# pixeli99/SVD_Xtend

Measured on AMD Instinct MI355X. Metric: train-step samples/sec (14-frame 512x320 fp16 SVD UNet), higher is better.
Workload: dtype fp16; 1 GPU; SVD UNet train step, 14 frames 512x320, batch 1/GPU, 1524623082 params (397620480 trainable: temporal_transformer_block*), fwd + EDM loss + bwd + grad all-reduce + AdamW; global_batch=1, grad_accum=1, parallelism=dp1, grad_allreduce=none, ranks_seen=1, allreduce_bytes=1590482176, exec=hipgraph, gemm_tuning_sweeps=0, gemm_variant=4

## Files before the change

svd_xtend_amd/csrc/norm.hip:

```cpp
#include "common.h"
#include <stdlib.h>

namespace {


struct GnGeom {
    int n_s, rows, C, G, cg, cc, rpi;
    int slab;
};

__device__ __forceinline__ void group_sums(const float* stats, int n_s, int n, int G, int g, float i0, float i1, float& s, float& ss) {
    long long a = 0, b = 0;
    const long long* st = reinterpret_cast<const long long*>(stats);
#pragma unroll
    for (int r = 0; r < SVDX_GN_REPLICAS; ++r) {
        const size_t o = (((size_t)r * n_s + n) * G + g) * 2;
        a += st[o]; b += st[o + 1];
    }
    s = (float)a * i0; ss = (float)b * i1;
}
__device__ __forceinline__ void group_mean_rstd(const float* stats, int n_s, int n, int G, int g, float cnt, float eps, float i0, float i1,
                                                float& mean, float& rstd) {
    float s, ss;
    group_sums(stats, n_s, n, G, g, i0, i1, s, ss);
    mean = s / cnt;
    const float var = fmaxf(ss / cnt - mean * mean, 0.f);
    rstd = rsqrtf(var + eps);
}

template <bool BWD>
__device__ __forceinline__ void gn_block_stats(const float* stats, const float* bstats, const GnGeom& q, int n, float eps, float* sm) {
    const int g = threadIdx.x;
    if (g < q.G) {
        int fk0, fk1, bk0, bk1;
        gn_fixed_scales((long)q.rows * q.cg, 0, fk0, fk1);
        const float cnt = (float)q.rows * q.cg;
        float mean, rstd;
        group_mean_rstd(stats, q.n_s, n, q.G, g, cnt, eps, exp2f((float)-fk0), exp2f((float)-fk1), mean, rstd);
        sm[g * 4] = mean; sm[g * 4 + 1] = rstd;
        if (BWD) {
            gn_fixed_scales((long)q.rows * q.cg, 1, bk0, bk1);
            float s1, s2;
            group_sums(bstats, q.n_s, n, q.G, g, exp2f((float)-bk0), exp2f((float)-bk1), s1, s2);
            sm[g * 4 + 2] = s1 / cnt; sm[g * 4 + 3] = s2 / cnt;
        }
    }
    __syncthreads();
}
__device__ __forceinline__ void gn_load8f(const float* p, float (&o)[8]) {
    const f32x4 a = *reinterpret_cast<const f32x4*>(p), b = *reinterpret_cast<const f32x4*>(p + 4);
    o[0] = a[0]; o[1] = a[1]; o[2] = a[2]; o[3] = a[3]; o[4] = b[0]; o[5] = b[1]; o[6] = b[2]; o[7] = b[3];
}

template <typename T, int MODE>
__global__ void gn_reduce_kernel(const T* __restrict__ x, const T* __restrict__ dy, const float* __restrict__ stats,
                                 const float* __restrict__ gamma, const float* __restrict__ beta, float* out,
                                 GnGeom q, float eps, int silu) {
    __shared__ unsigned long long gacc[64];
    __shared__ float sm[32 * 4];
    const int t = threadIdx.x;
    if (t < 64) gacc[t] = 0ull;
    int sk0, sk1;
    gn_fixed_scales((long)q.rows * q.cg, MODE, sk0, sk1);
    const float m0 = exp2f((float)sk0), m1 = exp2f((float)sk1);
    const int n = blockIdx.x, slab = blockIdx.y;
    const int j = t % q.cc, ry = t / q.cc;
    const bool worker = ry < q.rpi;
    const int r0 = slab * q.slab, r1 = min(q.rows, r0 + q.slab);
    constexpr int U = MODE == 0 ? 4 : 2;
    const size_t base = (size_t)n * q.rows * q.C + j * 8;
    Vec8<T> xb[U], db[U], xn[U], dn[U];
    auto fetch = [&](int r, Vec8<T> (&xo)[U], Vec8<T> (&dd)[U]) __attribute__((always_inline)) {
#pragma unroll
        for (int u = 0; u < U; ++u) {
            const int rr = min(r + u * q.rpi, q.rows - 1);
            xo[u] = *reinterpret_cast<const Vec8<T>*>(x + base + (size_t)rr * q.C);
            if (MODE == 1) dd[u] = *reinterpret_cast<const Vec8<T>*>(dy + base + (size_t)rr * q.C);
        }
    };
    int r = r0 + ry;
    if (worker && r < r1) fetch(r, xb, db);
    float a0[8], a1[8];
#pragma unroll
    for (int e = 0; e < 8; ++e) a0[e] = a1[e] = 0.f;
    float sc[8], sh[8], gm[8], mu[8], rs[8];
    if (MODE == 1) {
        gn_block_stats<false>(stats, nullptr, q, n, eps, sm);
        float bt[8];
        gn_load8f(gamma + j * 8, gm);
        gn_load8f(beta + j * 8, bt);
#pragma unroll
        for (int e = 0; e < 8; ++e) {
            const int g = (j * 8 + e) / q.cg;
            mu[e] = sm[g * 4]; rs[e] = sm[g * 4 + 1];
            sc[e] = rs[e] * gm[e];
            sh[e] = bt[e] - mu[e] * sc[e];
        }
    } else {
        __syncthreads();
    }
    if (worker) {
        for (; r < r1; r += U * q.rpi) {
            const int rn = r + U * q.rpi;
            if (rn < r1) fetch(rn, xn, dn);
#pragma unroll
            for (int u = 0; u < U; ++u) {
                if (r + u * q.rpi < r1) {
                    if (MODE == 0) {
#pragma unroll
                        for (int e = 0; e < 8; ++e) { const float xv = to_f<T>(xb[u].v[e]); a0[e] += xv; a1[e] += xv * xv; }
                    } else {
#pragma unroll
                        for (int e = 0; e < 8; ++e) {
                            const float xv = to_f<T>(xb[u].v[e]);
                            float dz = to_f<T>(db[u].v[e]);
                            if (silu) dz *= silu_gradf_(xv * sc[e] + sh[e]);
                            const float dzg = dz * gm[e];
                            a0[e] += dzg;
                            a1[e] += dzg * (xv - mu[e]) * rs[e];
                        }
                    }
                }
            }
#pragma unroll
            for (int u = 0; u < U; ++u) { xb[u] = xn[u]; if (MODE == 1) db[u] = dn[u]; }
        }
        int cur = (j * 8) / q.cg;
        float s0 = 0.f, s1 = 0.f;
#pragma unroll
        for (int e = 0; e < 8; ++e) {
            const int g = (j * 8 + e) / q.cg;
            if (g != cur) {
                atomicAdd(&gacc[cur * 2], (unsigned long long)__float2ll_rn(s0 * m0));
                atomicAdd(&gacc[cur * 2 + 1], (unsigned long long)__float2ll_rn(s1 * m1));
                cur = g; s0 = 0.f; s1 = 0.f;
            }
            s0 += a0[e]; s1 += a1[e];
        }
        atomicAdd(&gacc[cur * 2], (unsigned long long)__float2ll_rn(s0 * m0));
        atomicAdd(&gacc[cur * 2 + 1], (unsigned long long)__float2ll_rn(s1 * m1));
    }
    __syncthreads();
    if (t < 2 * q.G)
        atomicAdd(reinterpret_cast<unsigned long long*>(out) + ((size_t)(slab % SVDX_GN_REPLICAS) * q.n_s + n) * q.G * 2 + t, gacc[t]);
}

template <typename T, int MODE>
__global__ void gn_apply_kernel(const T* __restrict__ x, const T* __restrict__ dy, const float* __restrict__ stats,
                                const float* __restrict__ bstats, const float* __restrict__ gamma,
                                const float* __restrict__ beta, const T* __restrict__ add, T* __restrict__ out,
                                GnGeom q, float eps, int silu) {
    __shared__ float sm[32 * 4];
    const int t = threadIdx.x;
    const int n = blockIdx.x, slab = blockIdx.y;
    const int j = t % q.cc, ry = t / q.cc;
    const bool worker = ry < q.rpi;
    const int r0 = slab * q.slab, r1 = min(q.rows, r0 + q.slab);
    constexpr int U = MODE == 0 ? 4 : 2;
    const size_t base = (size_t)n * q.rows * q.C + j * 8;
    Vec8<T> xb[U], db[U], ab[U], xn[U], dn[U], an[U];
    auto fetch = [&](int r, Vec8<T> (&xo)[U], Vec8<T> (&dd)[U], Vec8<T> (&aa)[U]) __attribute__((always_inline)) {
#pragma unroll
        for (int u = 0; u < U; ++u) {
            const size_t off = base + (size_t)min(r + u * q.rpi, q.rows - 1) * q.C;
            xo[u] = *reinterpret_cast<const Vec8<T>*>(x + off);
            if (MODE == 1) {
                dd[u] = *reinterpret_cast<const Vec8<T>*>(dy + off);
                if (add) aa[u] = *reinterpret_cast<const Vec8<T>*>(add + off);
            }
        }
    };
    int r = r0 + ry;
    if (worker && r < r1) fetch(r, xb, db, ab);
    gn_block_stats<MODE == 1>(stats, bstats, q, n, eps, sm);
    if (!worker) return;
    float sc[8], sh[8], gm[8], mu[8], rs[8], b1[8], b2[8], bt[8];
    gn_load8f(gamma + j * 8, gm);
    gn_load8f(beta + j * 8, bt);
#pragma unroll
    for (int e = 0; e < 8; ++e) {
        const int g = (j * 8 + e) / q.cg;
        mu[e] = sm[g * 4]; rs[e] = sm[g * 4 + 1];
        sc[e] = rs[e] * gm[e];
        sh[e] = bt[e] - mu[e] * sc[e];
        if (MODE == 1) { b1[e] = sm[g * 4 + 2]; b2[e] = sm[g * 4 + 3]; }
    }
    for (; r < r1; r += U * q.rpi) {
        const int rn = r + U * q.rpi;
        if (MODE == 0 && rn < r1) fetch(rn, xn, dn, an);
#pragma unroll
        for (int u = 0; u < U; ++u) {
            const int rr = r + u * q.rpi;
            if (rr < r1) {
                float o[8];
                if (MODE == 0) {
#pragma unroll
                    for (int e = 0; e < 8; ++e) {
                        const float z = to_f<T>(xb[u].v[e]) * sc[e] + sh[e];
                        o[e] = silu ? siluf_(z) : z;
                    }
                } else {
#pragma unroll
                    for (int e = 0; e < 8; ++e) {
                        const float xv = to_f<T>(xb[u].v[e]);
                        float dz = to_f<T>(db[u].v[e]);
                        if (silu) dz *= silu_gradf_(xv * sc[e] + sh[e]);
                        const float xhat = (xv - mu[e]) * rs[e];
                        o[e] = rs[e] * (dz * gm[e] - (b1[e] + xhat * b2[e]));
                        if (add) o[e] += to_f<T>(ab[u].v[e]);
                    }
                }
                store8<T>(out + base + (size_t)rr * q.C, o);
            }
        }
        if (MODE == 0) {
#pragma unroll
            for (int u = 0; u < U; ++u) xb[u] = xn[u];
        } else if (rn < r1) {
            fetch(rn, xb, db, ab);
        }
    }
}

int gn_geom(GnGeom& q, int n_s, int rows, int C, int G, int& threads, bool reduce = false) {
    SVDX_CHECK_ARG(n_s > 0 && rows > 0 && C > 0 && G > 0 && G <= 32, "groupnorm: bad sizes");
    SVDX_CHECK_ARG(C % G == 0 && C % 8 == 0 && C / 8 <= 1024, "groupnorm: C=%d must be a multiple of 8 and of G", C);
    q.n_s = n_s; q.rows = rows; q.C = C; q.G = G; q.cg = C / G; q.cc = C / 8;
    q.rpi = q.cc >= 256 ? 1 : 256 / q.cc;
    threads = q.cc * q.rpi;
    int slab = reduce ? 64 : 32;
    const long want = reduce ? 512 : 1024;
    while (slab > 2 * q.rpi && slab > 2 && (long)n_s * ((rows + slab - 1) / slab) < want) slab >>= 1;
    q.slab = slab;
    return 0;
}

constexpr int LN_MAXCH_LIMIT = 4;

template <typename T, int LN_MAXCH, int R>
__global__ __launch_bounds__(256) void ln_fwd_kernel(const T* __restrict__ x, const float* __restrict__ gamma,
                                                     const float* __restrict__ beta, T* __restrict__ y,
                                                     float* __restrict__ stats, int rows, int C, float eps) {
    const int lane = threadIdx.x & 63;
    const int cc = C / 8;
    const int wid = blockIdx.x * 4 + (threadIdx.x >> 6), nw = gridDim.x * 4;
    const float invC = 1.f / (float)C;
    for (int row0 = wid * R; row0 < rows; row0 += nw * R) {
        Vec8<T> raw[R][LN_MAXCH];
#pragma unroll
        for (int k = 0; k < R; ++k) {
            const int row = min(row0 + k, rows - 1);
#pragma unroll
            for (int i = 0; i < LN_MAXCH; ++i) {
                const int j = lane + i * 64;
                if (j < cc) raw[k][i] = *reinterpret_cast<const Vec8<T>*>(x + (size_t)row * C + j * 8);
            }
        }
#pragma unroll
        for (int k = 0; k < R; ++k) {
            const int row = row0 + k;
            float v[LN_MAXCH][8];
            float s = 0.f;
#pragma unroll
            for (int i = 0; i < LN_MAXCH; ++i) {
                if (lane + i * 64 < cc) {
#pragma unroll
                    for (int e = 0; e < 8; ++e) { v[i][e] = to_f<T>(raw[k][i].v[e]); s += v[i][e]; }
                }
            }
            const float mean = wave_sum(s) * invC;
            float ss = 0.f;
#pragma unroll
            for (int i = 0; i < LN_MAXCH; ++i) {
                if (lane + i * 64 < cc) {
#pragma unroll
                    for (int e = 0; e < 8; ++e) { const float d = v[i][e] - mean; ss += d * d; }
                }
            }
            const float rstd = rsqrtf(wave_sum(ss) * invC + eps);
            if (row < rows) {
                if (lane == 0) { stats[(size_t)row * 2] = mean; stats[(size_t)row * 2 + 1] = rstd; }
#pragma unroll
                for (int i = 0; i < LN_MAXCH; ++i) {
                    const int j = lane + i * 64;
                    if (j < cc) {
                        float o[8];
#pragma unroll
                        for (int e = 0; e < 8; ++e) o[e] = (v[i][e] - mean) * rstd * gamma[j * 8 + e] + beta[j * 8 + e];
                        store8<T>(y + (size_t)row * C + j * 8, o);
                    }
                }
            }
        }
    }
}

template <typename T, int NCH>
__global__ __launch_bounds__(256) void ln_fwd16_kernel(const T* __restrict__ x, const float* __restrict__ gamma, const float* __restrict__ beta,
                                                       T* __restrict__ y, float* __restrict__ stats, int rows, int C, float eps) {
    const int l16 = threadIdx.x & 15, grp = threadIdx.x >> 4;
    const int cc = C / 8;
    float gm[NCH][8], bt[NCH][8];
    bool cv[NCH];
    int cl[NCH];
#pragma unroll
    for (int j = 0; j < NCH; ++j) {
        const int c = l16 + 16 * j;
        cv[j] = c < cc;
        cl[j] = min(c, cc - 1);
        gn_load8f(gamma + cl[j] * 8, gm[j]);
        gn_load8f(beta + cl[j] * 8, bt[j]);
    }
    const float invC = 1.f / (float)C;
    constexpr int R = 2;
    for (int row0 = (blockIdx.x * 16 + grp) * R; row0 < rows; row0 += gridDim.x * 16 * R) {
        Vec8<T> raw[R][NCH];
#pragma unroll
        for (int k = 0; k < R; ++k)
#pragma unroll
            for (int j = 0; j < NCH; ++j) raw[k][j] = *reinterpret_cast<const Vec8<T>*>(x + (size_t)min(row0 + k, rows - 1) * C + cl[j] * 8);
#pragma unroll
        for (int k = 0; k < R; ++k) {
            const int row = row0 + k;
            float v[NCH][8];
            float s = 0.f;
#pragma unroll
            for (int j = 0; j < NCH; ++j)
#pragma unroll
                for (int e = 0; e < 8; ++e) { v[j][e] = cv[j] ? to_f<T>(raw[k][j].v[e]) : 0.f; s += v[j][e]; }
            const float mean = row16_sum(s) * invC;
            float ss = 0.f;
#pragma unroll
            for (int j = 0; j < NCH; ++j)
#pragma unroll
                for (int e = 0; e < 8; ++e) { const float d = cv[j] ? v[j][e] - mean : 0.f; ss += d * d; }
            const float rstd = rsqrtf(row16_sum(ss) * invC + eps);
            if (row < rows) {
                if (l16 == 0) *reinterpret_cast<float2*>(stats + (size_t)row * 2) = float2{mean, rstd};
#pragma unroll
                for (int j = 0; j < NCH; ++j) {
                    if (cv[j]) {
                        float o[8];
#pragma unroll
                        for (int e = 0; e < 8; ++e) o[e] = (v[j][e] - mean) * rstd * gm[j][e] + bt[j][e];
                        store8<T>(y + (size_t)row * C + cl[j] * 8, o);
                    }
                }
            }
        }
    }
}

template <int LANES>
__device__ __forceinline__ float ln_group_sum(float v) {
    v = row16_sum(v);
    if (LANES >= 32) v += __shfl_xor(v, 16, 64);
    if (LANES >= 64) v += __shfl_xor(v, 32, 64);
    return v;
}

template <typename T, int LANES, int NCH, bool AFFINE>
__global__ __launch_bounds__(256, 2) void ln_bwd_kernel(const T* __restrict__ dy, const T* __restrict__ x, const float* __restrict__ stats,
                                                        const float* __restrict__ gamma, const T* __restrict__ add, const T* __restrict__ add2,
                                                        float add2_scale, T* __restrict__ dx, float* dgamma, float* dbeta, float* partial, int rows,
                                                        int C) {
    extern __shared__ float red[];
    constexpr int GROUPS = 256 / LANES;
    const int ll = threadIdx.x % LANES, grp = threadIdx.x / LANES;
    const int cc = C / 8;
    float gm[NCH][8], pg[AFFINE ? NCH : 1][8], pb[AFFINE ? NCH : 1][8];
    bool cv[NCH];
    int cl[NCH];
#pragma unroll
    for (int j = 0; j < NCH; ++j) {
        const int c = ll + LANES * j;
        cv[j] = c < cc;
        cl[j] = min(c, cc - 1);
        gn_load8f(gamma + cl[j] * 8, gm[j]);
        if (AFFINE) {
#pragma unroll
            for (int e = 0; e < 8; ++e) pg[j][e] = pb[j][e] = 0.f;
        }
    }
    const float invC = 1.f / (float)C;
    for (int row = blockIdx.x * GROUPS + grp; row < rows; row += gridDim.x * GROUPS) {
        constexpr bool PRE = !(AFFINE && NCH > 3);
        Vec8<T> xr[NCH], dr[NCH], ar[PRE ? NCH : 1], a2r[PRE ? NCH : 1];
#pragma unroll
        for (int j = 0; j < NCH; ++j) {
            if (cv[j]) {
                const size_t off = (size_t)row * C + cl[j] * 8;
                xr[j] = *reinterpret_cast<const Vec8<T>*>(x + off);
                dr[j] = *reinterpret_cast<const Vec8<T>*>(dy + off);
                if (PRE && add) ar[j] = *reinterpret_cast<const Vec8<T>*>(add + off);
                if (PRE && add2) a2r[j] = *reinterpret_cast<const Vec8<T>*>(add2 + off);
            }
        }
        const float2 mr = *reinterpret_cast<const float2*>(stats + (size_t)row * 2);
        float s1 = 0.f, s2 = 0.f;
#pragma unroll
        for (int j = 0; j < NCH; ++j) {
            if (cv[j]) {
#pragma unroll
                for (int e = 0; e < 8; ++e) {
                    const float d = to_f<T>(dr[j].v[e]);
                    const float xh = (to_f<T>(xr[j].v[e]) - mr.x) * mr.y;
                    const float dg = d * gm[j][e];
                    s1 += dg;
                    s2 += dg * xh;
                    if (AFFINE) {
                        pg[j][e] += d * xh;
                        pb[j][e] += d;
                    }
                }
            }
        }
        const float m1 = ln_group_sum<LANES>(s1) * invC, m2 = ln_group_sum<LANES>(s2) * invC;
#pragma unroll
        for (int j = 0; j < NCH; ++j) {
            if (cv[j]) {
                const size_t off = (size_t)row * C + cl[j] * 8;
                float o[8];
#pragma unroll
                for (int e = 0; e < 8; ++e) {
                    const float xh = (to_f<T>(xr[j].v[e]) - mr.x) * mr.y;
                    o[e] = mr.y * (to_f<T>(dr[j].v[e]) * gm[j][e] - m1 - xh * m2);
                }
                if (add) {
                    const Vec8<T> a8 = PRE ? ar[PRE ? j : 0] : *reinterpret_cast<const Vec8<T>*>(add + off);
#pragma unroll
                    for (int e = 0; e < 8; ++e) o[e] += to_f<T>(a8.v[e]);
                }
                if (add2) {
                    const Vec8<T> a8 = PRE ? a2r[PRE ? j : 0] : *reinterpret_cast<const Vec8<T>*>(add2 + off);
#pragma unroll
                    for (int e = 0; e < 8; ++e) o[e] += add2_scale * to_f<T>(a8.v[e]);
                }
                store8<T>(dx + off, o);
            }
        }
    }
    if (AFFINE) {
        float* mine = red + (size_t)grp * C;
#pragma unroll 1
        for (int which = 0; which < 2; ++which) {
#pragma unroll
            for (int j = 0; j < NCH; ++j) {
                if (cv[j]) {
#pragma unroll
                    for (int e = 0; e < 8; ++e) mine[cl[j] * 8 + e] = which == 0 ? pg[j][e] : pb[j][e];
                }
            }
            __syncthreads();
            for (int i = threadIdx.x; i < C; i += 256) {
                float t = 0.f;
#pragma unroll
                for (int g = 0; g < GROUPS; ++g) t += red[(size_t)g * C + i];
                if (partial) partial[(size_t)blockIdx.x * 2 * C + which * C + i] = t;
                else atomicAdd((which == 0 ? dgamma : dbeta) + i, t);
            }
            __syncthreads();
        }
    }
}

__device__ __forceinline__ void ln_param_reduce_body(const float* __restrict__ partial, int nblk, int C, float* dgamma, float* dbeta,
                                                     int blk, float (*sm)[64]) {
    const int cl = threadIdx.x & 63, rg = threadIdx.x >> 6;
    const int col = blk * 64 + cl;
    float s = 0.f;
    if (col < 2 * C) {
#pragma unroll 8
        for (int b = rg; b < nblk; b += 16) s += partial[(size_t)b * 2 * C + col];
    }
    sm[rg][cl] = s;
    __syncthreads();
    if (rg == 0 && col < 2 * C) {
        float t = 0.f;
#pragma unroll
        for (int i = 0; i < 16; ++i) t += sm[i][cl];
        if (col < C) dgamma[col] += t; else dbeta[col - C] += t;
    }
}

__global__ __launch_bounds__(1024) void ln_param_reduce_kernel(const float* __restrict__ partial, int nblk, int C,
                                                               float* dgamma, float* dbeta) {
    __shared__ float sm[16][64];
    ln_param_reduce_body(partial, nblk, C, dgamma, dbeta, blockIdx.x, sm);
}

struct LnRedPack {
    svdx_lnred_job job[SVDX_BATCH_MAX_JOBS];
    int start[SVDX_BATCH_MAX_JOBS + 1];
    int n_jobs;
};

__global__ __launch_bounds__(1024) void ln_param_reduce_batch_kernel(const LnRedPack pk) {
    __shared__ float sm[16][64];
    int j = 0;
    while (j + 1 < pk.n_jobs && (int)blockIdx.x >= pk.start[j + 1]) ++j;
    const svdx_lnred_job& q = pk.job[j];
    ln_param_reduce_body(q.partial, q.nblk, q.C, q.dgamma, q.dbeta, blockIdx.x - pk.start[j], sm);
}

static int ln_bwd_affine_blocks(int rows, int C) {
    const int cc = C / 8;
    const int lanes = cc <= 48 ? 16 : (cc <= 96 ? 32 : 64);
    const int groups = 256 / lanes;
    const int per = 1;
    const int cap = min(512, SVDX_LN_PARTIAL_ROWS);
    return max(1, min(cdiv(rows, per * groups), cap));
}

}

extern "C" int svdx_ln_bwd_blocks(int rows, int C) { return rows > 0 && C > 0 && C % 8 == 0 ? ln_bwd_affine_blocks(rows, C) : 0; }

extern "C" int svdx_ln_param_reduce_batch(const svdx_lnred_job* jobs, int n_jobs, void* stream) {
    SVDX_CHECK_ARG(jobs && n_jobs > 0, "svdx_ln_param_reduce_batch: bad args");
    for (int j0 = 0; j0 < n_jobs; j0 += SVDX_BATCH_MAX_JOBS) {
        LnRedPack pk;
        pk.n_jobs = min(n_jobs - j0, SVDX_BATCH_MAX_JOBS);
        int blocks = 0;
        for (int j = 0; j < pk.n_jobs; ++j) {
            const svdx_lnred_job& q = jobs[j0 + j];
            SVDX_CHECK_ARG(q.partial && q.dgamma && q.dbeta && q.nblk > 0 && q.C > 0, "svdx_ln_param_reduce_batch: job %d: bad args", j0 + j);
            pk.job[j] = q;
            pk.start[j] = blocks;
            blocks += cdiv(2 * q.C, 64);
        }
        for (int j = pk.n_jobs; j <= SVDX_BATCH_MAX_JOBS; ++j) pk.start[j] = blocks;
        hipLaunchKernelGGL(ln_param_reduce_batch_kernel, dim3(blocks), dim3(1024), 0, (hipStream_t)stream, pk);
        SVDX_LAUNCH_CHECK("svdx_ln_param_reduce_batch");
    }
    return 0;
}

extern "C" int svdx_gn_stats(const void* x, float* stats, int n_s, int rows, int C, int G, int prezeroed, int dtype, void* stream) {
    GnGeom q; int threads;
    if (int rc = gn_geom(q, n_s, rows, C, G, threads, true)) return rc;
    hipStream_t st = (hipStream_t)stream;
    if (!prezeroed) { if (int rc = svdx_zero(stats, sizeof(long long) * 2 * n_s * G * SVDX_GN_REPLICAS, stream)) return rc; }
    dim3 grid(n_s, cdiv(rows, q.slab));
    DISPATCH_DTYPE(dtype, hipLaunchKernelGGL((gn_reduce_kernel<T, 0>), grid, dim3(threads), 0, st, (const T*)x,
                                             (const T*)nullptr, (const float*)nullptr, (const float*)nullptr,
                                             (const float*)nullptr, stats, q, 0.f, 0));
    SVDX_LAUNCH_CHECK("svdx_gn_stats");
    return 0;
}

extern "C" int svdx_gn_apply(const void* x, const float* stats, const float* gamma, const float* beta, void* y,
                             int n_s, int rows, int C, int G, float eps, int silu, int dtype, void* stream) {
    GnGeom q; int threads;
    if (int rc = gn_geom(q, n_s, rows, C, G, threads)) return rc;
    dim3 grid(n_s, cdiv(rows, q.slab));
    DISPATCH_DTYPE(dtype, hipLaunchKernelGGL((gn_apply_kernel<T, 0>), grid, dim3(threads), 0, (hipStream_t)stream,
                                             (const T*)x, (const T*)nullptr, stats, (const float*)nullptr, gamma, beta,
                                             (const T*)nullptr, (T*)y, q, eps, silu));
    SVDX_LAUNCH_CHECK("svdx_gn_apply");
    return 0;
}

extern "C" int svdx_gn_bwd_stats(const void* dy, const void* x, const float* stats, const float* gamma,
                                 const float* beta, float* bstats, int n_s, int rows, int C, int G, float eps,
                                 int silu, int prezeroed, int dtype, void* stream) {
    GnGeom q; int threads;
    if (int rc = gn_geom(q, n_s, rows, C, G, threads, true)) return rc;
    hipStream_t st = (hipStream_t)stream;
    if (!prezeroed) { if (int rc = svdx_zero(bstats, sizeof(long long) * 2 * n_s * G * SVDX_GN_REPLICAS, stream)) return rc; }
    dim3 grid(n_s, cdiv(rows, q.slab));
    DISPATCH_DTYPE(dtype, hipLaunchKernelGGL((gn_reduce_kernel<T, 1>), grid, dim3(threads), 0, st, (const T*)x,
                                             (const T*)dy, stats, gamma, beta, bstats, q, eps, silu));
    SVDX_LAUNCH_CHECK("svdx_gn_bwd_stats");
    return 0;
}

extern "C" int svdx_gn_bwd_apply(const void* dy, const void* x, const float* stats, const float* bstats,
                                 const float* gamma, const float* beta, const void* add, void* dx, int n_s, int rows,
                                 int C, int G, float eps, int silu, int dtype, void* stream) {
    GnGeom q; int threads;
    if (int rc = gn_geom(q, n_s, rows, C, G, threads)) return rc;
    dim3 grid(n_s, cdiv(rows, q.slab));
    DISPATCH_DTYPE(dtype, hipLaunchKernelGGL((gn_apply_kernel<T, 1>), grid, dim3(threads), 0, (hipStream_t)stream,
                                             (const T*)x, (const T*)dy, stats, bstats, gamma, beta, (const T*)add,
                                             (T*)dx, q, eps, silu));
    SVDX_LAUNCH_CHECK("svdx_gn_bwd_apply");
    return 0;
}

extern "C" int svdx_ln_fwd(const void* x, const float* gamma, const float* beta, void* y, float* stats, int rows,
                           int C, float eps, int dtype, void* stream) {
    SVDX_CHECK_ARG(rows > 0 && C % 8 == 0 && C / 8 <= 64 * LN_MAXCH_LIMIT, "svdx_ln_fwd: C=%d unsupported", C);
    const int nch16 = (C / 8 + 15) / 16;
    if (nch16 <= 5) {
        const int blocks16 = min(cdiv(rows, 32), 2048);
#define LN_FWD16(NCH) hipLaunchKernelGGL((ln_fwd16_kernel<T, NCH>), dim3(blocks16), dim3(256), 0, (hipStream_t)stream, (const T*)x, gamma, beta, \
                                         (T*)y, stats, rows, C, eps)
        DISPATCH_DTYPE(dtype, { if (nch16 == 1) LN_FWD16(1); else if (nch16 == 2) LN_FWD16(2); else if (nch16 == 3) LN_FWD16(3); else LN_FWD16(5); });
#undef LN_FWD16
        SVDX_LAUNCH_CHECK("svdx_ln_fwd");
        return 0;
    }
    const int nch = (C / 8 + 63) / 64;
    const int R = nch == 1 ? 4 : (nch == 2 ? 2 : 1);
    const int blocks = min(cdiv(rows, 4 * R), 4096);
#define LN_FWD(NCH, RR) hipLaunchKernelGGL((ln_fwd_kernel<T, NCH, RR>), dim3(blocks), dim3(256), 0, (hipStream_t)stream, (const T*)x, gamma, \
                                           beta, (T*)y, stats, rows, C, eps)
    DISPATCH_DTYPE(dtype, { if (nch == 1) LN_FWD(1, 4); else if (nch == 2) LN_FWD(2, 2); else if (nch == 3) LN_FWD(3, 1); else LN_FWD(4, 1); });
#undef LN_FWD
    SVDX_LAUNCH_CHECK("svdx_ln_fwd");
    return 0;
}

extern "C" int svdx_ln_bwd(const void* dy, const void* x, const float* stats, const float* gamma, const void* add, const void* add2,
                           float add2_scale, void* dx, float* dgamma, float* dbeta, float* scratch, int rows, int C, int defer_reduce,
                           int dtype, void* stream) {
    SVDX_CHECK_ARG(rows > 0 && C % 8 == 0 && C / 8 <= 64 * LN_MAXCH_LIMIT, "svdx_ln_bwd: C=%d unsupported", C);
    SVDX_CHECK_ARG((dgamma == nullptr) == (dbeta == nullptr), "svdx_ln_bwd: dgamma/dbeta must come together");
    hipStream_t st = (hipStream_t)stream;
    const int cc = C / 8;
    const int lanes = cc <= 48 ? 16 : (cc <= 96 ? 32 : 64);
    const int nch = (cc + lanes - 1) / lanes;
    const int groups = 256 / lanes;
    SVDX_CHECK_ARG(!defer_reduce || (dgamma && scratch), "svdx_ln_bwd: defer_reduce needs dgamma/dbeta and scratch");
    int blocks = min(cdiv(rows, groups), 2048);
    if (dgamma) blocks = scratch ? ln_bwd_affine_blocks(rows, C) : min(blocks, 256);
    const size_t sh = dgamma ? sizeof(float) * groups * C : 0;
    SVDX_CHECK_ARG(sh <= 64 * 1024, "svdx_ln_bwd: C=%d too wide for the affine-gradient slab", C);
#define LN_BWD_A(L, N, A)                                                                                                          \
    hipLaunchKernelGGL((ln_bwd_kernel<T, L, N, A>), dim3(blocks), dim3(256), sh, st, (const T*)dy, (const T*)x, stats, gamma,           \
                       (const T*)add, (const T*)add2, add2_scale, (T*)dx, dgamma, dbeta, scratch, rows, C)
#define LN_BWD(L, N)                                                                                                                  \
    {                                                                                                                                 \
        if (dgamma) LN_BWD_A(L, N, true); else LN_BWD_A(L, N, false);                                                                   \
    }
    DISPATCH_DTYPE(dtype, {
        if (lanes == 16) { if (nch == 1) LN_BWD(16, 1) else if (nch == 2) LN_BWD(16, 2) else LN_BWD(16, 3) }
        else if (lanes == 32) LN_BWD(32, 3)
        else { if (nch <= 3) LN_BWD(64, 3) else LN_BWD(64, 4) }
    });
#undef LN_BWD
#undef LN_BWD_A
    SVDX_LAUNCH_CHECK("svdx_ln_bwd");
    if (dgamma && scratch && !defer_reduce) {
        hipLaunchKernelGGL(ln_param_reduce_kernel, dim3(cdiv(2 * C, 64)), dim3(1024), 0, st, scratch, blocks, C, dgamma, dbeta);
        SVDX_LAUNCH_CHECK("svdx_ln_bwd(param reduce)");
    }
    return 0;
}
```

Measured before the change: 21.44 samples/s.

## Prefetch next row in LN backward, hoist LN gamma/beta, merge affine reductions

```diff
diff --git a/svd_xtend_amd/csrc/norm.hip b/svd_xtend_amd/csrc/norm.hip
--- a/svd_xtend_amd/csrc/norm.hip
+++ b/svd_xtend_amd/csrc/norm.hip
@@ -85,10 +85,10 @@
     for (int e = 0; e < 8; ++e) a0[e] = a1[e] = 0.f;
     float sc[8], sh[8], gm[8], mu[8], rs[8];
     if (MODE == 1) {
-        gn_block_stats<false>(stats, nullptr, q, n, eps, sm);
         float bt[8];
         gn_load8f(gamma + j * 8, gm);
         gn_load8f(beta + j * 8, bt);
+        gn_block_stats<false>(stats, nullptr, q, n, eps, sm);
 #pragma unroll
         for (int e = 0; e < 8; ++e) {
             const int g = (j * 8 + e) / q.cg;
@@ -172,11 +172,11 @@
     };
     int r = r0 + ry;
     if (worker && r < r1) fetch(r, xb, db, ab);
-    gn_block_stats<MODE == 1>(stats, bstats, q, n, eps, sm);
-    if (!worker) return;
     float sc[8], sh[8], gm[8], mu[8], rs[8], b1[8], b2[8], bt[8];
     gn_load8f(gamma + j * 8, gm);
     gn_load8f(beta + j * 8, bt);
+    gn_block_stats<MODE == 1>(stats, bstats, q, n, eps, sm);
+    if (!worker) return;
 #pragma unroll
     for (int e = 0; e < 8; ++e) {
         const int g = (j * 8 + e) / q.cg;
@@ -245,6 +245,13 @@
     const int cc = C / 8;
     const int wid = blockIdx.x * 4 + (threadIdx.x >> 6), nw = gridDim.x * 4;
     const float invC = 1.f / (float)C;
+    float gm[LN_MAXCH][8], bt[LN_MAXCH][8];
+#pragma unroll
+    for (int i = 0; i < LN_MAXCH; ++i) {
+        const int j = min(lane + i * 64, cc - 1);
+        gn_load8f(gamma + j * 8, gm[i]);
+        gn_load8f(beta + j * 8, bt[i]);
+    }
     for (int row0 = wid * R; row0 < rows; row0 += nw * R) {
         Vec8<T> raw[R][LN_MAXCH];
 #pragma unroll
@@ -286,7 +293,7 @@
                     if (j < cc) {
                         float o[8];
 #pragma unroll
-                        for (int e = 0; e < 8; ++e) o[e] = (v[i][e] - mean) * rstd * gamma[j * 8 + e] + beta[j * 8 + e];
+                        for (int e = 0; e < 8; ++e) o[e] = (v[i][e] - mean) * rstd * gm[i][e] + bt[i][e];
                         store8<T>(y + (size_t)row * C + j * 8, o);
                     }
                 }
@@ -383,28 +390,39 @@
         }
     }
     const float invC = 1.f / (float)C;
-    for (int row = blockIdx.x * GROUPS + grp; row < rows; row += gridDim.x * GROUPS) {
-        constexpr bool PRE = !(AFFINE && NCH > 3);
-        Vec8<T> xr[NCH], dr[NCH], ar[PRE ? NCH : 1], a2r[PRE ? NCH : 1];
+    constexpr bool PRE = !(AFFINE && NCH > 3);
+    constexpr bool AHEAD = AFFINE && NCH <= 3;
+    struct RowOps { Vec8<T> xr[NCH], dr[NCH]; float2 mr; };
+    struct RowAdds { Vec8<T> ar[PRE ? NCH : 1], a2r[PRE ? NCH : 1]; };
+    auto fetch_adds = [&](int row, int j, RowAdds& o) __attribute__((always_inline)) {
+        if (PRE && cv[j]) {
+            const size_t off = (size_t)row * C + cl[j] * 8;
+            if (add) o.ar[PRE ? j : 0] = *reinterpret_cast<const Vec8<T>*>(add + off);
+            if (add2) o.a2r[PRE ? j : 0] = *reinterpret_cast<const Vec8<T>*>(add2 + off);
+        }
+    };
+    auto fetch = [&](int row, RowOps& o, RowAdds* oa) __attribute__((always_inline)) {
 #pragma unroll
         for (int j = 0; j < NCH; ++j) {
             if (cv[j]) {
                 const size_t off = (size_t)row * C + cl[j] * 8;
-                xr[j] = *reinterpret_cast<const Vec8<T>*>(x + off);
-                dr[j] = *reinterpret_cast<const Vec8<T>*>(dy + off);
-                if (PRE && add) ar[j] = *reinterpret_cast<const Vec8<T>*>(add + off);
-                if (PRE && add2) a2r[j] = *reinterpret_cast<const Vec8<T>*>(add2 + off);
-            }
-        }
-        const float2 mr = *reinterpret_cast<const float2*>(stats + (size_t)row * 2);
+                o.xr[j] = *reinterpret_cast<const Vec8<T>*>(x + off);
+                o.dr[j] = *reinterpret_cast<const Vec8<T>*>(dy + off);
+            }
+            if (oa) fetch_adds(row, j, *oa);
+        }
+        o.mr = *reinterpret_cast<const float2*>(stats + (size_t)row * 2);
+    };
+    auto process = [&](int row, const RowOps& o, const RowAdds& oa) __attribute__((always_inline)) {
+        const float2 mr = o.mr;
         float s1 = 0.f, s2 = 0.f;
 #pragma unroll
         for (int j = 0; j < NCH; ++j) {
             if (cv[j]) {
 #pragma unroll
                 for (int e = 0; e < 8; ++e) {
-                    const float d = to_f<T>(dr[j].v[e]);
-                    const float xh = (to_f<T>(xr[j].v[e]) - mr.x) * mr.y;
+                    const float d = to_f<T>(o.dr[j].v[e]);
+                    const float xh = (to_f<T>(o.xr[j].v[e]) - mr.x) * mr.y;
                     const float dg = d * gm[j][e];
                     s1 += dg;
                     s2 += dg * xh;
@@ -420,46 +438,70 @@
         for (int j = 0; j < NCH; ++j) {
             if (cv[j]) {
                 const size_t off = (size_t)row * C + cl[j] * 8;
-                float o[8];
+                float v[8];
 #pragma unroll
                 for (int e = 0; e < 8; ++e) {
-                    const float xh = (to_f<T>(xr[j].v[e]) - mr.x) * mr.y;
-                    o[e] = mr.y * (to_f<T>(dr[j].v[e]) * gm[j][e] - m1 - xh * m2);
+                    const float xh = (to_f<T>(o.xr[j].v[e]) - mr.x) * mr.y;
+                    v[e] = mr.y * (to_f<T>(o.dr[j].v[e]) * gm[j][e] - m1 - xh * m2);
                 }
                 if (add) {
-                    const Vec8<T> a8 = PRE ? ar[PRE ? j : 0] : *reinterpret_cast<const Vec8<T>*>(add + off);
-#pragma unroll
-                    for (int e = 0; e < 8; ++e) o[e] += to_f<T>(a8.v[e]);
+                    const Vec8<T> a8 = PRE ? oa.ar[PRE ? j : 0] : *reinterpret_cast<const Vec8<T>*>(add + off);
+#pragma unroll
+                    for (int e = 0; e < 8; ++e) v[e] += to_f<T>(a8.v[e]);
                 }
                 if (add2) {
-                    const Vec8<T> a8 = PRE ? a2r[PRE ? j : 0] : *reinterpret_cast<const Vec8<T>*>(add2 + off);
-#pragma unroll
-                    for (int e = 0; e < 8; ++e) o[e] += add2_scale * to_f<T>(a8.v[e]);
-                }
-                store8<T>(dx + off, o);
-            }
+                    const Vec8<T> a8 = PRE ? oa.a2r[PRE ? j : 0] : *reinterpret_cast<const Vec8<T>*>(add2 + off);
+#pragma unroll
+                    for (int e = 0; e < 8; ++e) v[e] += add2_scale * to_f<T>(a8.v[e]);
+                }
+                store8<T>(dx + off, v);
+            }
+        }
+    };
+    int row = blockIdx.x * GROUPS + grp;
+    if (AHEAD) {
+        RowOps a, b;
+        RowAdds ad;
+        if (row < rows) fetch(row, a, nullptr);
+        while (row < rows) {
+            int nrow = row + gridDim.x * GROUPS;
+#pragma unroll
+            for (int j = 0; j < NCH; ++j) fetch_adds(row, j, ad);
+            if (nrow < rows) fetch(nrow, b, nullptr);
+            process(row, a, ad);
+            row = nrow;
+            if (row >= rows) break;
+            nrow = row + gridDim.x * GROUPS;
+#pragma unroll
+            for (int j = 0; j < NCH; ++j) fetch_adds(row, j, ad);
+            if (nrow < rows) fetch(nrow, a, nullptr);
+            process(row, b, ad);
+            row = nrow;
+        }
+    } else {
+        for (; row < rows; row += gridDim.x * GROUPS) {
+            RowOps a;
+            RowAdds ad;
+            fetch(row, a, &ad);
+            process(row, a, ad);
         }
     }
     if (AFFINE) {
-        float* mine = red + (size_t)grp * C;
-#pragma unroll 1
-        for (int which = 0; which < 2; ++which) {
-#pragma unroll
-            for (int j = 0; j < NCH; ++j) {
-                if (cv[j]) {
-#pragma unroll
-                    for (int e = 0; e < 8; ++e) mine[cl[j] * 8 + e] = which == 0 ? pg[j][e] : pb[j][e];
-                }
-            }
-            __syncthreads();
-            for (int i = threadIdx.x; i < C; i += 256) {
-                float t = 0.f;
-#pragma unroll
-                for (int g = 0; g < GROUPS; ++g) t += red[(size_t)g * C + i];
-                if (partial) partial[(size_t)blockIdx.x * 2 * C + which * C + i] = t;
-                else atomicAdd((which == 0 ? dgamma : dbeta) + i, t);
-            }
-            __syncthreads();
+        float* mine = red + (size_t)grp * 2 * C;
+#pragma unroll
+        for (int j = 0; j < NCH; ++j) {
+            if (cv[j]) {
+#pragma unroll
+                for (int e = 0; e < 8; ++e) { mine[cl[j] * 8 + e] = pg[j][e]; mine[C + cl[j] * 8 + e] = pb[j][e]; }
+            }
+        }
+        __syncthreads();
+        for (int i = threadIdx.x; i < 2 * C; i += 256) {
+            float t = 0.f;
+#pragma unroll
+            for (int g = 0; g < GROUPS; ++g) t += red[(size_t)g * 2 * C + i];
+            if (partial) partial[(size_t)blockIdx.x * 2 * C + i] = t;
+            else atomicAdd(i < C ? dgamma + i : dbeta + (i - C), t);
         }
     }
 }
@@ -625,7 +667,7 @@
     SVDX_CHECK_ARG(!defer_reduce || (dgamma && scratch), "svdx_ln_bwd: defer_reduce needs dgamma/dbeta and scratch");
     int blocks = min(cdiv(rows, groups), 2048);
     if (dgamma) blocks = scratch ? ln_bwd_affine_blocks(rows, C) : min(blocks, 256);
-    const size_t sh = dgamma ? sizeof(float) * groups * C : 0;
+    const size_t sh = dgamma ? sizeof(float) * groups * 2 * C : 0;
     SVDX_CHECK_ARG(sh <= 64 * 1024, "svdx_ln_bwd: C=%d too wide for the affine-gradient slab", C);
 #define LN_BWD_A(L, N, A)                                                                                                          \
     hipLaunchKernelGGL((ln_bwd_kernel<T, L, N, A>), dim3(blocks), dim3(256), sh, st, (const T*)dy, (const T*)x, stats, gamma,           \
```

New measurement: 21.43 samples/s, median of 3. No clear change (-0.0%).
